# cirKITers/qml-essentials

Measured on AMD Instinct MI355X. Metric: gate_applies_per_s, higher is better.
Workload: dtype complex64

## Files before the change

### qml-essentials_amd/csrc/qmle_engine.hip

```cpp
#include <hip/hip_runtime.h>

#include <cmath>
#include <cstdio>
#include <cstdlib>
#include <cstring>
#include <algorithm>
#include <atomic>
#include <new>
#include <utility>

#include "qmle_internal.h"
#include "qmle_host.h"
#include "qmle_dev.h"
#include "qmle_matrices.h"

#include <map>
#include <mutex>
#include <vector>

namespace {

template <bool GMAJOR>
__global__ void __launch_bounds__(64)
k_build_matrices(const BuildOp *__restrict__ build, const BuildGroup *__restrict__ groups, int n_groups,
// ... 806 lines not shown
    const float *mats = d_mats + (size_t)b0 * plan->mat_floats;
    const float *ang = d_angles ? d_angles + (size_t)b0 * plan->n_slots : nullptr;
    float2 *cols = d_cols ? d_cols + (size_t)b0 * plan->fold_groups * 16 : nullptr;
    bool initialised = false;
    TileRoute route;
    for (size_t si = 0; si < plan->stages.size(); ++si) {
      const Stage &st = plan->stages[si];
      const ChunkPipeline::StageQueued stage_queued = pipe.begin_stage(chunk_no, si);
      ProfScope prof_scope(plan, (int)si, stream);
      if (st.kind == ST_TILE) {
        const bool last = si + 1 == plan->stages.size();
        const bool last_mw = fuse_mw && last, last_fused = !fuse_mw && fuse_expval && last;
        const TileBuffers tb{stc, mats, ang, last_mw || last_fused ? d_partial : nullptr, last_fused ? obs_masks : nullptr,
                             cols, d_coef + (size_t)b0 * 32};
        TileRequest rq;
        rq.batch = bc;
        rq.init_zero = !initialised;
        rq.meas = last_mw ? TM_STORE_MW : !last_fused ? TM_STORE : by_position ? TM_EXPVAL_PARTIAL : TM_EXPVAL_MASKS;
        rq.n_obs = last_fused ? n_obs : 0;
        rq.from_zero = true;
        rq.fold_cols = cols != nullptr;
        rq.multi_rows = last_mw || (last_fused && (oc.single_bits || rq.meas == TM_EXPVAL_MASKS));
        rq.semi_single = oc.semi_single;
        const bool reuse = !last_mw && si == 0 && reuse_zeros;
        if (reuse) rq.zeroed_states = slot_zeroed[slot];
        rc = launch_tile(plan, si, tb, rq, stream, &route);
        note_product_form(plan, si, route, meas_type);
        if (last_fused && !is_reg_measure(route.family)) {
          plan->last_run.measure_tpw = 1 << route.row_shift;
          plan->last_run.measure_regs = route.from_regs;
          plan->last_run.wave_private = route.wave_private;
          plan->last_run.staging_dma = (route.walk & kWalkDma) != 0;
          plan->last_run.lane_swap = (route.walk & kWalkLaneSwap) != 0;
        }
        if (reuse && route.fill) {
          slot_zeroed[slot] = bc;
          filled_states += (uint64_t)bc;
        }
        if (reuse && route.fill_elided) elided = true;
        initialised = true;
      } else {
        if (!initialised) {
          launch_init_zero(stc, n, bc, stream);
          initialised = true;
        }
        rc = run_stage_inplace(plan, st, stc, mats, ang, bc, stream);
      }
      if (rc != QMLE_OK) return rc;
    }
    if (!initialised) launch_init_zero(stc, n, bc, stream);
    if (meas_type == QMLE_MEAS_PROBS) {
      const uint64_t tc = (uint64_t)bc * (D / 2);
      launch_probs(stc, (float *)d_out + (size_t)b0 * D, tc, stream);
    } else if (meas_type == QMLE_MEAS_EXPVAL_Z && fuse_expval) {
      const bool reg_measure = is_reg_measure(route.family);
      const int tiles = (1 << (n - plan->stages.back().T)) >> route.row_shift;
      launch_expval_final((const float *)d_partial, tiles, bc, n_obs, by_position && !reg_measure ? oc.by_position : oc.by_index,
                          (float *)d_out + (size_t)b0 * n_obs, stream);
    } else if (meas_type == QMLE_MEAS_EXPVAL_Z) {
      rc = oc.single_bits
               ? run_expval(stc, n, bc, oc.by_position.bits, n_obs, (float *)d_out + (size_t)b0 * n_obs,
                            d_partial, L.partial_bytes, stream)
               : run_parity_pos(stc, n, bc, obs_masks, n_obs, (float *)d_out + (size_t)b0 * n_obs,
                                d_partial, L.partial_bytes, stream);
      if (rc != QMLE_OK) return rc;
    } else if (meas_type == QMLE_MEAS_MEYER_WALLACH) {
// ... 371 lines not shown
```

### qml-essentials_amd/csrc/qmle_host.h

```cpp
#pragma once
#include <hip/hip_runtime.h>

#include <cstddef>
#include <cstdint>

#include "qmle_internal.h"

namespace qmle {

struct ObsBits {
  int8_t bits[QMLE_MAX_QUBITS] = {};
  uint32_t row_mask[QMLE_MAX_QUBITS] = {};
};

enum TileMeas : int {
  TM_STORE = 0,
  TM_PROBS = 1,
  TM_EXPVAL = 2,
  TM_EXPVAL_PARTIAL = 3,
  TM_EXPVAL_MASKS = 4,
  TM_STORE_MW = 5,
  TM_MW_ONLY = 6,
};

// ... 52 lines not shown
int tile_threads(int T);
constexpr uint32_t kWalkSlab = 1u, kWalkSyncStaged = 2u, kWalkSyncTileEnd = 4u, kWalkDma = 8u, kWalkLaneSwap = 16u,
                   kWalkLaneSwapCross = 32u;
struct TileRequest {
  int batch = 1;
  bool init_zero = false;
  int meas = TM_STORE;
  int n_obs = 0;
  bool from_zero = false;
  bool fold_cols = false;
  bool multi_rows = false;
  int zeroed_states = 0;
  bool semi_single = false;
  bool no_multi_zin = false;
  bool no_mw_lean = false;
};
struct TileRoute {
  int status = QMLE_OK;
  TileFamily family = TF_TILE;
  bool dense4 = false, mw = false;
  bool measure = false, multi = false, ws = false, masks = false;
  int mono_q = 0;
  bool pair = false;
  bool nt = false;
  unsigned grid_x = 1, grid_y = 1, threads = 64;
  size_t lds_bytes = 0;
  bool compact = false;
  uint32_t tile_free = 0;
  bool mw_lean = false, slots_in_lds = false;
  bool fill = false, fill_elided = false;
  int tpw = 1, row_shift = 0;
  uint32_t walk = 0;
  bool from_regs = false, wave_private = false, product_form = false;
};
TileRoute route_tile(const qmle_plan *p, size_t stage, const TileRequest &rq);
struct TileBuffers {
  float2 *states = nullptr;
  const float *mats = nullptr, *angles = nullptr;
  void *out = nullptr;
  const uint32_t *obs_masks = nullptr;
  float2 *cols = nullptr;
  float *coef = nullptr;
};
int launch_tile(const qmle_plan *p, size_t stage, const TileBuffers &b, TileRequest rq, hipStream_t stream,
                TileRoute *taken = nullptr);

int launch_direct(const qmle_plan *p, const LoweredOp &op, float2 *states, const float *mats,
                  int batch, hipStream_t stream);
void launch_init_zero(float2 *states, int n, int batch, hipStream_t stream);
void launch_diag_all(float2 *states, int n, int batch, const float *marks, const float *angles,
                     int n_slots, int slot, hipStream_t stream);
void launch_fill_zero(float2 *states, uint64_t n_float4, hipStream_t stream);

int expval_blocks(int n);
int overlap_blocks(int n);
int run_expval(const float2 *states, int n, int batch, const int8_t *obs_bits, int n_obs,
               float *d_out, void *ws, size_t ws_bytes, hipStream_t stream);
int run_parity_pos(const float2 *states, int n, int batch, const uint32_t *pos_masks, int n_obs,
                   float *d_out, void *ws, size_t ws_bytes, hipStream_t stream);
void launch_expval_final(const float *partial, int n_rows, int batch, int n_obs, const ObsBits &ob,
                         float *d_out, hipStream_t stream);
void launch_probs(const float2 *states, float *d_out, uint64_t total_chunks, hipStream_t stream);
void launch_density(const float2 *states, float2 *d_out, int n, int batch, hipStream_t stream);
bool mw_fusable(int n, const Stage &last);
bool mw_lean(int n, const Stage &last);
bool mw_lean_layout(int n, const Stage &last);
// ... 26 lines not shown
```

### qml-essentials_amd/csrc/qmle_internal.h

```cpp
#pragma once
#include <cstdint>
#include <string>
#include <vector>

#include "qmle_sv.h"

namespace qmle {


enum LKind : uint8_t {
  LK_1Q = 0,
  LK_2Q = 1,
  LK_DIAG_ALL = 2,
  LK_4Q = 3
};
enum LFlag : uint8_t {
  LF_DIAG = 1,
  LF_PERMX = 2,
  LF_PHASE = 4,
};

enum GKind : uint8_t {
  GK_SWEEP = 0,
  GK_REG4 = 1,
// ... 117 lines not shown
};
static inline ZregRecord zreg_record(uint16_t r) {
  return {(uint32_t)r & 15u, ((uint32_t)r >> 4) & 63u, ((uint32_t)r >> 10) & 31u, (uint32_t)r >> 15};
}

struct StageProfile {
  bool on = false;
  std::vector<void *> start, stop;
  std::vector<int> stage;
  size_t used = 0;
};

struct DevicePlan {
  int device = -1;
  void *blob = nullptr;
  size_t blob_bytes = 0;
  LoweredOp *d_ops = nullptr;
  OpGroup *d_op_groups = nullptr;
  BuildOp *d_build = nullptr;
  BuildGroup *d_groups = nullptr;
  float *d_consts = nullptr;
  LoweredOp *d_ops2 = nullptr;
  Group2 *d_groups2 = nullptr;
  uint32_t *d_tbl2 = nullptr;
};

enum { kChunkLoopNone = 0, kChunkLoopOneStream, kChunkLoopStaged, kChunkLoopFree };
constexpr const char *kChunkLoopNames[] = {"none", "one_stream", "staged", "free"};

struct LastRun {
  uint64_t stage0_written = 0;
  int measure_tpw = 0;
  bool measure_regs = false, wave_private = false, staging_dma = false, lane_swap = false;
  int chunk_loop = kChunkLoopNone;
  uint64_t product_form_stages = 0;
  bool matrices_from_map = false;
  bool measured_form = false;
};

}

struct qmle_plan {
  int n = 0, n_slots = 0;
  unsigned flags = 0;
  std::vector<qmle_op> ops;
  std::vector<float> consts;
  std::vector<qmle::LoweredOp> lowered;
  std::vector<std::vector<int>> lowered_src;
  std::vector<qmle::LoweredOp> dev_ops;
  std::vector<int> dev_src;
  std::vector<qmle::OpGroup> op_groups;
  std::vector<qmle::LoweredOp> ops2;
  std::vector<uint8_t> ops2_perm_tail;
  std::vector<qmle::Group2> groups2;
  std::vector<uint32_t> tbl2;
  std::vector<qmle::BuildOp> build_ops;
  std::vector<qmle::BuildGroup> groups;
  int n_groups_needed = 0;
  int n_product_groups = 0;
  std::vector<qmle::Stage> stages;
  uint32_t mat_floats = 0;
  uint32_t mat_floats_unit = 0;
  uint32_t mat_floats_old = 0;
  int fold_groups = 0;
  double model_cost = 0.0;
  int chosen_candidate = -1;
// ... 58 lines not shown
```

### qml-essentials_amd/csrc/qmle_plan.cpp

```cpp
#include <algorithm>
#include <cstdio>
#include <cstdlib>
#include <cstring>
#include <cmath>
#include <functional>
#include <sstream>

#include "qmle_internal.h"

namespace qmle {

namespace {

struct OpInfo {
  int n_wires;
  int n_params;
  bool has_const;
};

bool op_info(int opcode, OpInfo *info) {
  switch (opcode) {
    case QMLE_OP_ID: case QMLE_OP_X: case QMLE_OP_Y: case QMLE_OP_Z:
    case QMLE_OP_H: case QMLE_OP_S:
      *info = {1, 0, false}; return true;
// ... 1783 lines not shown
    describe_measuring(os, p, s);
    if (st.kind == ST_TILE) {
      os << ",\"unit_form_ops\":[";
      for (size_t i = 0; i < st.unit_form_ops.size(); ++i) os << (i ? "," : "") << st.unit_form_ops[i];
      os << "],\"scale_carriers\":[";
      for (size_t i = 0; i < st.scale_carriers.size(); ++i) os << (i ? "," : "") << st.scale_carriers[i];
      os << "],\"fast_ops\":[";
      if (st.fast_ok && st.fast_end > st.fast_begin) {
        uint32_t k = p->groups2[st.fast_begin].op_begin;
        bool any = false;
        for (int g = st.fast_begin; g < st.fast_end; ++g)
          for (int j = 0; j < (int)p->groups2[g].n_ops; ++j, ++k, any = true)
            os << (any ? "," : "") << "[" << (int)p->ops2[k].pad << "," << p->ops2[k].mat_off << "]";
      }
      os << "],\"product_form_groups\":[";
      for (int g = st.fast_begin; g < st.fast_end; ++g)
        os << (g > st.fast_begin ? "," : "") << ((p->groups2[g].sync & kGroupProduct) ? "true" : "false");
      os << "],\"product_form_records\":[";
      for (int g = st.fast_begin; g < st.fast_end; ++g)
        os << (g > st.fast_begin ? "," : "") << ((p->groups2[g].sync & kGroupProduct) ? (long long)p->groups2[g].prod_off : -1ll);
      os << "],\"closing_free_groups\":[";
      for (int g = st.fast_begin; g < st.fast_end; ++g)
        os << (g > st.fast_begin ? "," : "") << ((p->groups2[g].sync & kGroupClosingFree) ? "true" : "false");
      os << "],\"group_product_form_last_run\":" << (s < 64 && ((p->last_run.product_form_stages >> s) & 1u) ? "true" : "false")
         << ",\"measured_form_last_run\":" << (s + 1 == p->stages.size() && p->last_run.measured_form ? "true" : "false");
    }
    if (s + 1 == p->stages.size())
      os << ",\"measure_tiles_per_workgroup_last_run\":" << p->last_run.measure_tpw
         << ",\"measured_from_registers_last_run\":" << (p->last_run.measure_regs ? "true" : "false")
         << ",\"wave_private_walk_last_run\":" << (p->last_run.wave_private ? "true" : "false")
         << ",\"staging_dma_last_run\":" << (p->last_run.staging_dma ? "true" : "false")
         << ",\"last_group_lane_swap_last_run\":" << (p->last_run.lane_swap ? "true" : "false")
         << ",\"chunk_loop_last_run\":\"" << kChunkLoopNames[p->last_run.chunk_loop] << "\""
         << ",\"matrices_from_map_last_run\":" << (p->last_run.matrices_from_map ? "true" : "false");
    os << ",\"src_ops\":[";
    for (size_t i = 0; i < st.src_ops.size(); ++i) os << (i ? "," : "") << st.src_ops[i];
    os << "]}";
  }
  os << "]";
  if (p->expval_child)
    os << ",\"absorbed_ops\":" << p->absorbed.size()
       << ",\"expval_plan\":" << describe_plan(p->expval_child);
  os << "}";
  return os.str();
}

}
```

### qml-essentials_amd/csrc/qmle_tile.hip

```cpp
#include <hip/hip_runtime.h>

#include <cmath>
#include <cstdio>
#include <cstdlib>
#include <cstring>
#include <algorithm>
#include <atomic>
#include <new>
#include <utility>

#include "qmle_internal.h"
#include "qmle_host.h"
#include "qmle_dev.h"
#include "qmle_tile_dev.h"

namespace {

template <bool DENSE4, bool MW = false>
__global__ void k_tile(const TileArgs a) {
  extern __shared__ float4 smem4[];
  float2 *s = reinterpret_cast<float2 *>(smem4);
  const int T = a.T, L = a.L;
  uint32_t *lut = reinterpret_cast<uint32_t *>(s + (1u << T));
  const uint32_t lut_n = (1u << (T - L)) < 4u ? 4u : (1u << (T - L));
// ... 854 lines not shown
  const int n_obs = a.n_obs;
  for (int k0 = 0; k0 < n_obs; k0 += 8) {
    float v[8];
#pragma unroll
    for (int k = 0; k < 8; ++k) {
      v[k] = 0.f;
      if (k0 + k < n_obs) {
        const uint32_t m = om[k0 + k];
        const uint32_t mu = (m >> (T - 3)) & 7u;
        float t = 0.f;
#pragma unroll
        for (int u = 0; u < 8; ++u) {
          const float d = (m & 1u) ? Df[u] : S[u];
          t += (__popc((uint32_t)u & mu) & 1) ? -d : d;
        }
        v[k] = (__popc((uint32_t)lane & (m >> 1) & 63u) & 1) ? -t : t;
      }
    }
    wave_sums_dpp63(v);
    if (lane == kWave - 1) {
#pragma unroll
      for (int k = 0; k < 8; ++k) red[(k0 + k) * nw + wv] = v[k];
    }
  }
  __syncthreads();
  if (tid < n_obs) {
    const uint32_t mw = om[tid] >> 7;
    float r = 0.f;
    for (int w = 0; w < nw; ++w) r += (__popc((uint32_t)w & mw) & 1) ? -red[tid * nw + w] : red[tid * nw + w];
    reinterpret_cast<float *>(a.out)[(size_t)b * n_obs + tid] = r;
  }
}

template <bool NT, bool MEASURE, bool MULTI, bool WS = false, bool MW = false, bool MASKS = false>
__global__ void __launch_bounds__(512) __attribute__((amdgpu_waves_per_eu(MASKS ? 4 : 5))) k_tile2(const TileArgs a, const Tile2Args f) {
  extern __shared__ float4 smem4[];
  float2 *s = reinterpret_cast<float2 *>(smem4);
  const int T = a.T;
  const uint32_t sbo = lds_offset_of(smem4);
  float *red = a.meas == TM_EXPVAL ? reinterpret_cast<float *>(s + (1u << T)) : reinterpret_cast<float *>(s);
  const int tid = threadIdx.x, nt = blockDim.x;
  const int b = blockIdx.y;
  const int tpw = MULTI ? f.tpw : 1;
  uint32_t tile = blockIdx.x * (uint32_t)tpw;
  if (!MULTI && a.compact) {
    uint32_t rest = tile, free_bits = a.tile_free;
    tile = 0;
    while (rest) {
      const uint32_t low = free_bits & (0u - free_bits);
      if (rest & 1u) tile |= low;
      free_bits ^= low;
      rest >>= 1;
    }
  }
  const uint32_t n_tiles = gridDim.x * (uint32_t)tpw;
  const size_t D = (size_t)1 << a.n;
  uint64_t base = tile2_base(a, f, tile);
  char *st = reinterpret_cast<char *>(a.states + (size_t)b * D + base);
  constexpr bool ZR = MEASURE && MULTI && !WS && !MW && !MASKS;
  const uint32_t walk = ZR ? f.walk : (kWalkSyncStaged | kWalkSyncTileEnd);
  const bool slab = ZR && (walk & kWalkSlab) != 0;
  const bool dma = ZR && (walk & kWalkDma) != 0;
  const uint32_t jl = slab ? (2u * (tid & (kWave - 1))) | ((uint32_t)(tid / kWave) << 10) : 2u * tid;
  const int ush = slab ? 7 : T - 3;
  uint32_t goff8;
  if (f.n_in_runs < 0) {
// ... 7 lines not shown
    goff8 = g << 3;
  }
  uint32_t uoff[8], soff[8];
#pragma unroll
  for (int u = 0; u < 8; ++u) {
    uoff[u] = f.uoff8[u];
    soff[u] = sw((uint32_t)u << ush) << 3;
  }
  const uint32_t sl = (sw(jl) << 3) + sbo;
  const float4 z4 = make_float4(0.f, 0.f, 0.f, 0.f);
  if (!MULTI && (a.init_zero ? base != 0 : (tile & a.zin_outer) != 0)) {
    if (MW) {
      if (a.meas == TM_STORE_MW) {
#pragma unroll
        for (int u = 0; u < 8; ++u) st4<NT>(reinterpret_cast<float4 *>(st + uoff[u] + goff8), z4);
      }
      float *po = reinterpret_cast<float *>(a.out) + ((size_t)b * n_tiles + tile) * kMwFusedRow;
      if (tid < kMwFusedRow) po[tid] = 0.f;
    } else if (!MEASURE && a.meas == TM_STORE) {
#pragma unroll
      for (int u = 0; u < 8; ++u) st4<NT>(reinterpret_cast<float4 *>(st + uoff[u] + goff8), z4);
    } else if (!MEASURE) {
      char *po = reinterpret_cast<char *>(reinterpret_cast<float *>(a.out) + (size_t)b * D + base);
#pragma unroll
      for (int u = 0; u < 8; ++u) *reinterpret_cast<float2 *>(po + (uoff[u] >> 1) + (goff8 >> 1)) = make_float2(0.f, 0.f);
    } else {
      float *po = reinterpret_cast<float *>(a.out) +
                  ((size_t)b * n_tiles + tile) * (QMLE_MAX_QUBITS + 1);
      if (tid <= QMLE_MAX_QUBITS) po[tid] = 0.f;
    }
    return;
  }
  auto dma_tile = [&](const char *p) {
    if constexpr (ZR) {
      const uint32_t wv = (uint32_t)__builtin_amdgcn_readfirstlane(tid / kWave);
      __attribute__((address_space(3))) char *slab0 =
          (__attribute__((address_space(3))) char *)reinterpret_cast<char *>(smem4) + (wv << 13);
      asm volatile("" : "+s"(p));
      uint32_t vo[4];
      static_for<4>([&](auto k) {
        vo[(int)k] = goff8 ^ f.dma_delta[(int)k];
        asm volatile("" : "+v"(vo[(int)k]));
      });
      static_for<8>([&](auto u) {
        const char *src = p + uoff[(int)u] + vo[(int)u & 3];
        __builtin_amdgcn_global_load_lds((const __attribute__((address_space(1))) void *)src, slab0 + ((int)u << 10), 16, 0,
                                         NT ? 2 : 0);
      });
    }
  };
  if (dma) dma_tile(st);
  const Group2 QMLE_CONSTANT *grp = as_constant(f.groups);
  const uint32_t addr = f.n_groups > 0 ? f.tbl[grp->tbl + tid] : 0u;
  const u64 QMLE_CONSTANT *mrow = as_constant(reinterpret_cast<const u64 *>(a.mats + (size_t)b * a.mat_floats));
  int qsrc = -1;
  if (MEASURE) {
    const int8_t QMLE_CONSTANT *ka = (const int8_t QMLE_CONSTANT *)__builtin_amdgcn_kernarg_segment_ptr();
    qsrc = tid <= QMLE_MAX_QUBITS ? (int)ka[offsetof(TileArgs, qsrc) + tid] : 64;
  }
  const bool plain = MULTI || (!a.init_zero && !a.zin_local);
  float4 v[8];
  const uint32_t zl_m = MULTI ? (a.zin_local & ~1u) : 0u;
  const bool z0_m = MULTI && (a.zin_local & 1u) != 0;
  auto load_tile = [&](const char *p) {
    if (MULTI && a.zin_local) {
#pragma unroll
      for (int u = 0; u < 8; ++u) {
        v[u] = z4;
        if (((jl | ((uint32_t)u << ush)) & zl_m) == 0) {
          v[u] = ld4<NT>(reinterpret_cast<const float4 *>(p + uoff[u] + goff8));
          if (z0_m) v[u].z = v[u].w = 0.f;
        }
      }
    } else {
#pragma unroll
      for (int u = 0; u < 8; ++u) v[u] = ld4<NT>(reinterpret_cast<const float4 *>(p + uoff[u] + goff8));
    }
  };
  if (plain && !ZR) load_tile(st);
  const uint32_t sl_outer = sl;
  float zsq[ZR ? 16 : 1], zwk[4] = {0.f, 0.f, 0.f, 0.f};
  if (ZR) static_for<16>([&](auto c) { zsq[ZR ? (int)c : 0] = 0.f; });
// ... 93 lines not shown
        }
      } else {
        float4 w[8];
#pragma unroll
        for (int u = 0; u < 8; ++u) w[u] = lds_ld128(sl ^ soff[u]);
#pragma unroll
        for (int u = 0; u < 8; ++u) st4<NT>(reinterpret_cast<float4 *>(st_cur + uoff[u] + goff8), w[u]);
      }
    } else {
      char *po = reinterpret_cast<char *>(reinterpret_cast<float *>(a.out) + (size_t)b * D + base_cur);
#pragma unroll
      for (int u = 0; u < 8; ++u) {
        const float4 w = lds_ld128(sl ^ soff[u]);
        *reinterpret_cast<float2 *>(po + (uoff[u] >> 1) + (goff8 >> 1)) =
            make_float2(w.x * w.x + w.y * w.y, w.z * w.z + w.w * w.w);
      }
    }
    if (ZR && !(walk & kWalkSyncTileEnd)) asm volatile("" ::: "memory");
    else if (i + 1 < tpw) __syncthreads();
  }
  if (MW)
    tile_mw_finish(macc, T, (uint32_t)tid, reinterpret_cast<float *>(s),
                   reinterpret_cast<float *>(a.out) + ((size_t)b * gridDim.x + blockIdx.x) * kMwFusedRow, a.mw_lean != 0);
  else if (MEASURE && MULTI && MASKS) {
    if constexpr (MASKS)
      tile_m_finish(reinterpret_cast<float *>(a.out), red, pacc, a.n_obs, m_ol, T, tid, nt, blockIdx.x, gridDim.x, b);
  } else if (MEASURE && MULTI) {
    if constexpr (ZR)
      tile_zr_finish(reinterpret_cast<float *>(a.out), red, zsq, zwk, m_ol, T, qsrc, tid, nt,
                     31 - __builtin_clz((unsigned)tpw), blockIdx.x, gridDim.x, b);
  }
}


template <bool FOLD>
__global__ void __launch_bounds__(1024) k_reg_measure(const TileArgs a, int q) {
  extern __shared__ float4 smem4[];
  OpSlot *slots = reinterpret_cast<OpSlot *>(smem4);
  uint32_t *meta = reinterpret_cast<uint32_t *>(slots + a.n_ops);
  uint32_t *m_thr = meta;
  uint32_t *m_reg = meta + 32;
  uint32_t *m_pack = meta + 64;
  uint32_t *flipF = meta + 68;
  uint32_t *flipP = meta + 100;
  float *red = reinterpret_cast<float *>(meta + 132);
  const int T = a.T, tid = threadIdx.x, b = blockIdx.y;
  const int n_outer = a.n - T;
  const OpGroup g = a.groups[0];
  const int b0 = g.bits[0], b1 = g.bits[1], b2 = g.bits[2], b3 = g.bits[3];

  tile_stage_slots(a, slots, b);
  if (tid < 32) {
    uint32_t mt = 0, mi = 0;
    if (tid < a.n_obs) {
      const uint32_t m = a.obs_mask[tid];
      int tb = 0;
      for (int j = 0; j < T; ++j) {
        const uint32_t bitv = (m >> a.tile_bits[j]) & 1u;
        if (j == b0) mi |= bitv;
        else if (j == b1) mi |= bitv << 1;
        else if (j == b2) mi |= bitv << 2;
        else if (j == b3) mi |= bitv << 3;
        else mt |= bitv << tb++;
      }
    }
    m_thr[tid] = mt;
// ... 496 lines not shown
}

namespace qmle {

size_t tile_lds_bytes(int T, int L, int n_slots) {
  const size_t lut_n = ((size_t)1 << (T - L)) < 4 ? 4 : ((size_t)1 << (T - L));
  return ((size_t)8 << T) + 4 * lut_n + 288 * sizeof(float) + (size_t)n_slots * sizeof(OpSlot);
}

int tile_threads(int T) {
  int t = T >= 4 ? 1 << (T - 4) : 64;
  if (t < 64) t = 64;
  if (t > 1024) t = 1024;
  return t;
}

#define QMLE_TILE2_INSTANCES(X)                    \
  X(false, false, false, false, false, false)      \
  X(true,  false, false, false, false, false)      \
  X(false, true,  false, false, false, false)      \
  X(true,  true,  false, false, false, false)      \
  X(false, false, true,  false, false, false)      \
  X(true,  false, true,  false, false, false)      \
  X(false, true,  true,  false, false, false)      \
  X(true,  true,  true,  false, false, false)      \
  X(false, true,  true,  false, false, true)       \
  X(true,  true,  true,  false, false, true)       \
  X(false, false, false, true,  false, false)      \
  X(false, true,  false, true,  false, false)      \
  X(false, true,  false, false, true,  false)      \
  X(true,  true,  false, false, true,  false)      \
  X(false, true,  false, true,  true,  false)
#define QMLE_TILE2(NT, ME, MU, WS, MW, MA) (k_tile2<NT, ME, MU, WS, MW, MA>)
#define QMLE_TILE_INSTANCES(X) X(false, false) X(true, false) X(false, true) X(true, true)
#define QMLE_TILE1(D4, MW) (k_tile<D4, MW>)

static TileRoute route_reg_measure(const qmle_plan *p, const Stage &st, TileFamily family, int batch) {
  TileRoute r;
  r.family = family;
  r.slots_in_lds = true;
  const int n_outer = p->n - st.T;
  int q = 0;
  while (q < 6 && q < n_outer && (((uint64_t)batch << n_outer) >> (q + 1)) >= 4096) ++q;
  r.threads = 1u << (st.T - 4);
  r.lds_bytes = (size_t)(st.op_end - st.op_begin) * sizeof(OpSlot) + (132 + 16 * 32 + 128) * sizeof(uint32_t);
  if (family == TF_REG_MEASURE_MONO) {
    q = 5;
    r.mono_q = 5;
    r.lds_bytes = 16 * 32 * sizeof(float);
    uint32_t zin_local = 0, zin_outer = 0;
    if (plan_sparse(p) && st.zero_in) stage_known_zeros(p, st, &zin_local, &zin_outer);
    const OpGroup &g = p->op_groups[st.grp_begin];
    if (g.bits[0] != 0 && st.tile_bits[0] == 0 && !(zin_local & 1u) && st.T >= 11 && n_outer >= 4) {
      q = 4;
      r.mono_q = 4;
      r.pair = true;
      r.threads = 1u << (st.T - 5);
      const int n_live = p->n - __builtin_popcount(st.zero_in);
      r.nt = ((uint64_t)batch << (n_live + 3)) >= (1ull << 30);
    }
  }
  r.grid_x = 1u << (n_outer - q);
  r.grid_y = (unsigned)batch;
  r.row_shift = q;
  r.tpw = 1 << q;
  return r;
}

TileRoute route_tile(const qmle_plan *p, size_t si, const TileRequest &rq) {
  const Stage &st = p->stages[si];
  const int meas = rq.meas, batch = rq.batch, n_obs = rq.n_obs;
  const bool init_zero = rq.init_zero;
  if ((meas == TM_EXPVAL_PARTIAL || meas == TM_EXPVAL_MASKS) && !init_zero && n_obs >= 1 && n_obs <= 32) {
    TileFamily k = expval_kernel_of(p, si, plan_sparse(p));
    if (k == TF_REG_MEASURE && rq.semi_single) k = TF_TILE;
    if (k != TF_TILE) return route_reg_measure(p, st, k, batch);
  }
  TileRoute r;
  const bool from_zero = rq.from_zero && plan_sparse(p);
  uint32_t zin_local = 0, zin_outer = 0;
  if (from_zero && st.zero_in && !init_zero) stage_known_zeros(p, st, &zin_local, &zin_outer);
  const int n_ops = st.op_end - st.op_begin;
  r.slots_in_lds = tile_lds_bytes(st.T, st.L, n_ops) <= 160 * 1024;
  r.nt = st.T < p->n && !(from_zero && st.zero_in) && !init_zero &&
         ((uint64_t)batch << (p->n + 3)) >= (1ull << 30);
  r.mw_lean = meas == TM_STORE_MW && !rq.no_mw_lean && mw_lean_layout(p->n, st);
  if ((meas == TM_STORE_MW || (meas == TM_STORE && !st.next_tile && !init_zero)) && st.T < p->n &&
      ((uint64_t)batch << (p->n + 3)) >= (1ull << 30))
    r.nt = true;
  for (int g = st.grp_begin; g < st.grp_end; ++g)
    r.dense4 |= p->op_groups[g].kind == GK_DENSE4 || p->op_groups[g].kind == GK_REG4X;
  const unsigned tiles = 1u << (p->n - st.T);
  const int threads = tile_threads(st.T);
  r.threads = (unsigned)threads;
  r.grid_x = tiles;
  r.grid_y = (unsigned)batch;
  if (init_zero && !from_zero && meas == TM_STORE && st.T < p->n && tiles > 1 &&
      (st.fast_ok || st.T == kLdsMaxQubits) && p->n <= 28 && threads == (1 << (st.T - 4))) {
    if (rq.zeroed_states >= batch) r.fill_elided = true;
// ... 58 lines not shown
        r.grid_x /= 2u;
      }
    }
    if ((meas == TM_EXPVAL_PARTIAL || meas == TM_EXPVAL_MASKS) && r.tpw > 1) {
      if (!rq.multi_rows || r.tpw > 8) {
        r.grid_x *= (unsigned)r.tpw;
        r.tpw = 1;
      } else {
        r.row_shift = 31 - __builtin_clz((unsigned)r.tpw);
      }
    }
    if (meas == TM_EXPVAL_PARTIAL && r.tpw > 1) {
      if (!st.zreg_ok) {
        r.status = QMLE_ERR_INTERNAL;
        return r;
      }
      r.from_regs = true;
      r.wave_private = st.wave_private;
      r.walk = (p->groups2[st.fast_begin].sync & 1 ? kWalkSyncStaged : 0u) | (st.sync_tile_end ? kWalkSyncTileEnd : 0u);
      if (st.slab_load) {
        r.walk |= kWalkSlab;
        const bool dma = walk_by_dma(st, zin_local);
        if (dma) r.walk |= kWalkDma;
        if (walk_by_lane_swap(st, dma)) r.walk |= kWalkLaneSwap | (st.lane_swap_cross ? kWalkLaneSwapCross : 0u);
      }
    }
    r.lds_bytes = ((size_t)8 << st.T) +
                  (meas == TM_EXPVAL ? (size_t)QMLE_MAX_QUBITS * (threads >= kWave ? threads / kWave : 1) * sizeof(float) : 0);
    r.measure = !(meas == TM_STORE || meas == TM_PROBS);
    r.multi = r.tpw > 1;
    r.mw = meas == TM_STORE_MW || meas == TM_MW_ONLY;
    r.ws = r.mw ? st.T == p->n : st.T == p->n && !r.multi && !r.nt;
    r.masks = !r.mw && !r.ws && r.measure && r.multi && meas == TM_EXPVAL_MASKS;
    return r;
  }
  r.lds_bytes = tile_lds_bytes(st.T, st.L, r.slots_in_lds ? n_ops : 0);
  if (meas == TM_STORE_MW || meas == TM_MW_ONLY) {
    if (st.T < 10 || threads != (1 << (st.T - 4))) {
      r.status = QMLE_ERR_UNSUPPORTED;
      return r;
    }
    r.mw = true;
  }
  return r;
}

namespace {

TileArgs route_tile_args(const qmle_plan *p, const Stage &st, const TileBuffers &b, const TileRequest &rq,
                         const TileRoute &r) {
  TileArgs a = fill_tile_args(p, st, b.states, b.mats, b.angles, rq.init_zero, rq.meas, b.out, b.obs_masks, rq.n_obs,
                              rq.from_zero && plan_sparse(p));
  a.slots_in_lds = r.slots_in_lds;
  a.nt = r.nt;
  a.mw_lean = r.mw_lean;
  a.compact = r.compact;
  a.tile_free = r.tile_free;
  return a;
}

int issue_reg_measure(const qmle_plan *p, const Stage &st, const TileBuffers &b, const TileRequest &rq,
                      const TileRoute &r, hipStream_t stream) {
  const int batch = rq.batch, n_obs = rq.n_obs, n_outer = p->n - st.T;
  TileArgs a = fill_tile_args(p, st, b.states, b.mats, b.angles, false, TM_EXPVAL_MASKS, b.out, b.obs_masks, n_obs,
                              plan_sparse(p));
  a.slots_in_lds = 1;
// ... 49 lines not shown
      for (int i = 0; i < 4; ++i)
        pa.gpos[g][i] = (uint32_t)st.tile_bits[p->op_groups[st.grp_begin + g].bits[i]];
    if (r.nt) hipLaunchKernelGGL(k_product_stream<true>, grid, block, 0, stream, pa);
    else hipLaunchKernelGGL(k_product_stream<false>, grid, block, 0, stream, pa);
  } else {
    const TileArgs a = route_tile_args(p, st, b, rq, r);
    const uint32_t n_tiles = r.compact ? 1u << __builtin_popcount(r.tile_free) : 1u << (p->n - st.T);
    hipLaunchKernelGGL(k_tile_product, grid, block, r.lds_bytes, stream, a, b.cols, r.tpw, n_tiles);
  }
  HIPCHK(hipGetLastError());
  return QMLE_OK;
}

int issue_tile(const qmle_plan *p, const Stage &st, const TileBuffers &b, const TileRequest &rq, const TileRoute &r,
               hipStream_t stream) {
  if (FirstUse once{0}; once.first) {
#define QMLE_X(D4, MW)                      \
  QMLE_LDS_BASE_CHECK(QMLE_TILE1(D4, MW)); \
  HIPCHK(hipFuncSetAttribute((const void *)QMLE_TILE1(D4, MW), hipFuncAttributeMaxDynamicSharedMemorySize, 160 * 1024));
    QMLE_TILE_INSTANCES(QMLE_X)
#undef QMLE_X
    once.done();
  }
  const TileArgs a = route_tile_args(p, st, b, rq, r);
  const dim3 grid(r.grid_x, r.grid_y), block(r.threads);
#define QMLE_X(D4, MW) \
  if (r.dense4 == D4 && r.mw == MW) hipLaunchKernelGGL(QMLE_TILE1(D4, MW), grid, block, r.lds_bytes, stream, a); else
  QMLE_TILE_INSTANCES(QMLE_X) return QMLE_ERR_INTERNAL;
#undef QMLE_X
  HIPCHK(hipGetLastError());
  return QMLE_OK;
}

int issue_tile2(const qmle_plan *p, const Stage &st, const TileBuffers &b, const TileRequest &rq, const TileRoute &r,
                hipStream_t stream) {
  if (FirstUse once{1}; once.first) {
#define QMLE_X(NT, ME, MU, WS, MW, MA)                      \
  QMLE_LDS_BASE_CHECK(QMLE_TILE2(NT, ME, MU, WS, MW, MA)); \
  HIPCHK(hipFuncSetAttribute((const void *)QMLE_TILE2(NT, ME, MU, WS, MW, MA), hipFuncAttributeMaxDynamicSharedMemorySize, 160 * 1024));
    QMLE_TILE2_INSTANCES(QMLE_X)
#undef QMLE_X
    once.done();
  }
  TileArgs a = route_tile_args(p, st, b, rq, r);
  Tile2Args f;
  f.groups = p->dev.d_groups2 + st.fast_begin;
  f.ops = p->dev.d_ops2;
  f.tbl = p->dev.d_tbl2;
  f.n_groups = st.fast_end - st.fast_begin;
  f.n_ops_stage = 0;
  for (int g = st.fast_begin; g < st.fast_end; ++g) f.n_ops_stage += p->groups2[g].n_ops;
  f.gtab = st.fast_gtab;
  {
    int nr = 0;
    const int n_outer = p->n - st.T;
    for (int i = 0; i < n_outer && nr <= 6;) {
      int len = 1;
      while (i + len < n_outer && st.outer_bits[i + len] == st.outer_bits[i] + len) ++len;
      if (nr < 6) {
        f.run_off[nr] = (uint32_t)i;
        f.run_mask[nr] = len >= 32 ? 0xffffffffu : ((1u << len) - 1u);
        f.run_pos[nr] = (uint32_t)st.outer_bits[i];
      }
      ++nr;
      i += len;
    }
    f.n_runs = nr <= 6 ? nr : -1;
    for (int k = nr < 6 ? nr : 6; k < 6; ++k) f.run_off[k] = f.run_mask[k] = f.run_pos[k] = 0;
  }
  auto lane_runs = [&](int top) { f.n_in_runs = stage_lane_runs(st, top, f.in_off, f.in_mask, f.in_pos); };
  lane_runs(st.T - 4);
  for (unsigned u = 0; u < 8; ++u)
    f.uoff8[u] = (((u & 1u) << st.tile_bits[st.T - 3]) | (((u >> 1) & 1u) << st.tile_bits[st.T - 2]) |
                  (((u >> 2) & 1u) << st.tile_bits[st.T - 1])) << 3;
  f.walk = r.walk;
  for (int k = 0; k < 4; ++k) f.dma_delta[k] = 0;
  f.tpw = r.tpw;
  f.tile_stride = r.tpw > 1 ? 1u << st.outer_bits[0] : 0u;
  if (r.from_regs) {
    static_assert(sizeof(st.zreg) <= sizeof(a.obs_local), "the records travel in TileArgs::obs_local");
    std::memcpy(a.obs_local, st.zreg, sizeof(st.zreg));
    for (int j = 0; j < st.T; ++j) a.qsrc[(int)st.tile_bits[j]] = (uint8_t)j;
    a.qsrc[QMLE_MAX_QUBITS] = (uint8_t)kZrTotal;
    if (r.walk & kWalkSlab) {
      f.gtab = st.fast_gtab_slab;
      lane_runs(st.T - 1);
      for (unsigned u = 0; u < 8; ++u)
        f.uoff8[u] = (((u & 1u) << st.tile_bits[7]) | (((u >> 1) & 1u) << st.tile_bits[8]) |
                      (((u >> 2) & 1u) << st.tile_bits[9])) << 3;
    }
    if (r.walk & kWalkDma) {
      f.gtab = st.fast_gtab_dma;
      for (int k = 0; k < 4; ++k) f.dma_delta[k] = st.dma_delta[k];
    }
    if (r.walk & kWalkLaneSwap) {
      static_assert(sizeof(st.zreg_swap) == sizeof(st.zreg), "one record layout");
      std::memcpy(a.obs_local, st.zreg_swap, sizeof(st.zreg_swap));
    }
  }
  const dim3 grid(r.grid_x, r.grid_y), block(r.threads);
#define QMLE_X(NT, ME, MU, WS, MW, MA)                                                                         \
  if (r.nt == NT && r.measure == ME && r.multi == MU && r.ws == WS && r.mw == MW && r.masks == MA)             \
    hipLaunchKernelGGL(QMLE_TILE2(NT, ME, MU, WS, MW, MA), grid, block, r.lds_bytes, stream, a, f);           \
  else
  QMLE_TILE2_INSTANCES(QMLE_X) return QMLE_ERR_INTERNAL;
#undef QMLE_X
  HIPCHK(hipGetLastError());
  return QMLE_OK;
}

}

int launch_tile(const qmle_plan *p, size_t stage, const TileBuffers &b, TileRequest rq, hipStream_t stream,
                TileRoute *taken) {
  const Stage &st = p->stages[stage];
  rq.no_multi_zin = std::getenv("QMLE_NO_MULTI_ZIN") != nullptr;
  rq.no_mw_lean = rq.meas == TM_STORE_MW && mw_no_lean_switch();
  const TileRoute r = route_tile(p, stage, rq);
  if (taken) *taken = r;
  if (r.status != QMLE_OK) return r.status;
  if (r.fill) launch_fill_zero(b.states, ((uint64_t)rq.batch << p->n) / 2u , stream);
  switch (r.family) {
    case TF_TILE: return issue_tile(p, st, b, rq, r, stream);
    case TF_TILE2: return issue_tile2(p, st, b, rq, r, stream);
    case TF_TILE_PRODUCT:
    case TF_PRODUCT_STREAM: return issue_product(p, st, b, rq, r, stream);
    default: return issue_reg_measure(p, st, b, rq, r, stream);
  }
}

}

int qmle_plan_tile_route(const qmle_plan *plan, int stage, int batch, int meas, int n_obs, unsigned request_flags,
                         char *buf, size_t cap) {
  using namespace qmle;
  if (!plan || stage < 0 || (size_t)stage >= plan->stages.size() || plan->stages[stage].kind != ST_TILE || batch < 1 ||
      batch > kMaxGridY || meas < TM_STORE || meas > TM_MW_ONLY || n_obs < 0 || n_obs > QMLE_MAX_QUBITS)
    return QMLE_ERR_INVALID_ARG;
  TileRequest rq;
  rq.batch = batch;
  rq.meas = meas;
  rq.n_obs = n_obs;
  rq.init_zero = request_flags & QMLE_ROUTE_INIT_ZERO;
  rq.from_zero = request_flags & QMLE_ROUTE_FROM_ZERO;
  rq.fold_cols = request_flags & QMLE_ROUTE_FOLD_COLS;
  rq.multi_rows = request_flags & QMLE_ROUTE_MULTI_ROWS;
  rq.zeroed_states = (request_flags & QMLE_ROUTE_ZEROS_IN_PLACE) ? batch : 0;
  rq.semi_single = request_flags & QMLE_ROUTE_SEMI_SINGLE;
  rq.no_multi_zin = request_flags & QMLE_ROUTE_NO_MULTI_ZIN;
  rq.no_mw_lean = request_flags & QMLE_ROUTE_NO_MW_LEAN;
  const TileRoute r = route_tile(plan, (size_t)stage, rq);
  auto tf = [](bool v) { return v ? "true" : "false"; };
  char js[1024];
  const int len = std::snprintf(
      js, sizeof(js),
      "{\"status\":%d,\"family\":\"%s\",\"dense4\":%s,\"mw\":%s,\"nt\":%s,\"measure\":%s,\"multi\":%s,\"ws\":%s,"
      "\"masks\":%s,\"mono_q\":%d,\"pair\":%s,\"grid\":[%u,%u],\"threads\":%u,\"lds_bytes\":%zu,\"compact\":%s,"
      "\"tile_free\":%u,\"mw_lean\":%s,\"slots_in_lds\":%s,\"fill\":%s,\"fill_elided\":%s,\"tiles_per_workgroup\":%d,"
      "\"row_shift\":%d,\"walk_slab\":%s,\"walk_sync_staged\":%s,\"walk_sync_tile_end\":%s,\"staging_dma\":%s,"
      "\"lane_swap\":%s,\"lane_swap_crossed\":%s,\"from_registers\":%s,\"wave_private\":%s,\"product_form\":%s}",
      r.status, kTileFamilyNames[r.family], tf(r.dense4), tf(r.mw), tf(r.nt), tf(r.measure), tf(r.multi), tf(r.ws),
      tf(r.masks), r.mono_q, tf(r.pair), r.grid_x, r.grid_y, r.threads, r.lds_bytes, tf(r.compact), r.tile_free,
      tf(r.mw_lean), tf(r.slots_in_lds), tf(r.fill), tf(r.fill_elided), r.tpw, r.row_shift, tf(r.walk & kWalkSlab),
      tf(r.walk & kWalkSyncStaged), tf(r.walk & kWalkSyncTileEnd), tf(r.walk & kWalkDma), tf(r.walk & kWalkLaneSwap),
      tf(r.walk & kWalkLaneSwapCross), tf(r.from_regs), tf(r.wave_private), tf(r.product_form));
  if (buf && cap > 0) {
    const size_t nc = (size_t)len < cap - 1 ? (size_t)len : cap - 1;
    std::memcpy(buf, js, nc);
    buf[nc] = 0;
  }
  return len;
}
```

Measured before the change: 4.005 million.

## Add specialized measure-walk kernel for DMA lane-swap register-measure tile stages

```diff
diff --git a/qml-essentials_amd/csrc/qmle_engine.hip b/qml-essentials_amd/csrc/qmle_engine.hip
--- a/qml-essentials_amd/csrc/qmle_engine.hip
+++ b/qml-essentials_amd/csrc/qmle_engine.hip
@@ -862,6 +862,7 @@
           plan->last_run.wave_private = route.wave_private;
           plan->last_run.staging_dma = (route.walk & kWalkDma) != 0;
           plan->last_run.lane_swap = (route.walk & kWalkLaneSwap) != 0;
+          plan->last_run.walk_kernel = route.walk_kernel;
         }
         if (reuse && route.fill) {
           slot_zeroed[slot] = bc;
diff --git a/qml-essentials_amd/csrc/qmle_host.h b/qml-essentials_amd/csrc/qmle_host.h
--- a/qml-essentials_amd/csrc/qmle_host.h
+++ b/qml-essentials_amd/csrc/qmle_host.h
@@ -108,6 +108,7 @@
   int tpw = 1, row_shift = 0;
   uint32_t walk = 0;
   bool from_regs = false, wave_private = false, product_form = false;
+  bool walk_kernel = false;
 };
 TileRoute route_tile(const qmle_plan *p, size_t stage, const TileRequest &rq);
 struct TileBuffers {
diff --git a/qml-essentials_amd/csrc/qmle_internal.h b/qml-essentials_amd/csrc/qmle_internal.h
--- a/qml-essentials_amd/csrc/qmle_internal.h
+++ b/qml-essentials_amd/csrc/qmle_internal.h
@@ -173,6 +173,7 @@
   uint64_t stage0_written = 0;
   int measure_tpw = 0;
   bool measure_regs = false, wave_private = false, staging_dma = false, lane_swap = false;
+  bool walk_kernel = false;
   int chunk_loop = kChunkLoopNone;
   uint64_t product_form_stages = 0;
   bool matrices_from_map = false;
diff --git a/qml-essentials_amd/csrc/qmle_plan.cpp b/qml-essentials_amd/csrc/qmle_plan.cpp
--- a/qml-essentials_amd/csrc/qmle_plan.cpp
+++ b/qml-essentials_amd/csrc/qmle_plan.cpp
@@ -1839,7 +1839,8 @@
          << ",\"staging_dma_last_run\":" << (p->last_run.staging_dma ? "true" : "false")
          << ",\"last_group_lane_swap_last_run\":" << (p->last_run.lane_swap ? "true" : "false")
          << ",\"chunk_loop_last_run\":\"" << kChunkLoopNames[p->last_run.chunk_loop] << "\""
-         << ",\"matrices_from_map_last_run\":" << (p->last_run.matrices_from_map ? "true" : "false");
+         << ",\"matrices_from_map_last_run\":" << (p->last_run.matrices_from_map ? "true" : "false")
+         << ",\"walk_kernel_last_run\":" << (p->last_run.walk_kernel ? "true" : "false");
     os << ",\"src_ops\":[";
     for (size_t i = 0; i < st.src_ops.size(); ++i) os << (i ? "," : "") << st.src_ops[i];
     os << "]}";
diff --git a/qml-essentials_amd/csrc/qmle_tile.hip b/qml-essentials_amd/csrc/qmle_tile.hip
--- a/qml-essentials_amd/csrc/qmle_tile.hip
+++ b/qml-essentials_amd/csrc/qmle_tile.hip
@@ -910,6 +910,25 @@
   }
 }
 
+template <bool NT>
+__device__ __forceinline__ void dma_tile_pieces(float4 *smem4, const char *p, int tid, uint32_t goff8,
+                                                const uint32_t (&uoff)[8], const uint32_t (&delta)[4]) {
+  const uint32_t wv = (uint32_t)__builtin_amdgcn_readfirstlane(tid / kWave);
+  __attribute__((address_space(3))) char *slab0 =
+      (__attribute__((address_space(3))) char *)reinterpret_cast<char *>(smem4) + (wv << 13);
+  asm volatile("" : "+s"(p));
+  uint32_t vo[4];
+  static_for<4>([&](auto k) {
+    vo[(int)k] = goff8 ^ delta[(int)k];
+    asm volatile("" : "+v"(vo[(int)k]));
+  });
+  static_for<8>([&](auto u) {
+    const char *src = p + uoff[(int)u] + vo[(int)u & 3];
+    __builtin_amdgcn_global_load_lds((const __attribute__((address_space(1))) void *)src, slab0 + ((int)u << 10), 16, 0,
+                                     NT ? 2 : 0);
+  });
+}
+
 template <bool NT, bool MEASURE, bool MULTI, bool WS = false, bool MW = false, bool MASKS = false>
 __global__ void __launch_bounds__(512) __attribute__((amdgpu_waves_per_eu(MASKS ? 4 : 5))) k_tile2(const TileArgs a, const Tile2Args f) {
   extern __shared__ float4 smem4[];
@@ -983,22 +1002,7 @@
     return;
   }
   auto dma_tile = [&](const char *p) {
-    if constexpr (ZR) {
-      const uint32_t wv = (uint32_t)__builtin_amdgcn_readfirstlane(tid / kWave);
-      __attribute__((address_space(3))) char *slab0 =
-          (__attribute__((address_space(3))) char *)reinterpret_cast<char *>(smem4) + (wv << 13);
-      asm volatile("" : "+s"(p));
-      uint32_t vo[4];
-      static_for<4>([&](auto k) {
-        vo[(int)k] = goff8 ^ f.dma_delta[(int)k];
-        asm volatile("" : "+v"(vo[(int)k]));
-      });
-      static_for<8>([&](auto u) {
-        const char *src = p + uoff[(int)u] + vo[(int)u & 3];
-        __builtin_amdgcn_global_load_lds((const __attribute__((address_space(1))) void *)src, slab0 + ((int)u << 10), 16, 0,
-                                         NT ? 2 : 0);
-      });
-    }
+    if constexpr (ZR) dma_tile_pieces<NT>(smem4, p, tid, goff8, uoff, f.dma_delta);
   };
   if (dma) dma_tile(st);
   const Group2 QMLE_CONSTANT *grp = as_constant(f.groups);
@@ -1158,6 +1162,114 @@
   }
 }
 
+struct WalkGroup {
+  uint32_t tbl;
+  uint32_t off[4];
+  uint32_t prod_off;
+  uint32_t flags;
+};
+struct WalkArgs {
+  const float2 *states;
+  const float *mats;
+  float *out;
+  const uint32_t *tbl;
+  uint32_t mat_floats;
+  int n, T, tpw;
+  uint32_t tile_stride;
+  int n_runs;
+  uint32_t run_off[6], run_mask[6], run_pos[6];
+  int n_in_runs;
+  uint32_t in_off[4], in_mask[4], in_pos[4], gtab;
+  uint32_t uoff8[8], dma_delta[4];
+  WalkGroup g[3];
+  uint32_t last_prod_off, last_low1;
+  uint16_t zreg[16];
+  uint8_t qsrc[QMLE_MAX_QUBITS + 1];
+};
+#define QMLE_WOFF(c, g) \
+  ((((c) & 1) ? (g).off[0] : 0u) ^ (((c) & 2) ? (g).off[1] : 0u) ^ (((c) & 4) ? (g).off[2] : 0u) ^ (((c) & 8) ? (g).off[3] : 0u))
+template <bool NT, int G, bool CROSS>
+__global__ void __launch_bounds__(512) __attribute__((amdgpu_waves_per_eu(5))) k_measure_walk(const WalkArgs w) {
+  static_assert(G >= 1 && G <= 3, "gathered groups");
+  extern __shared__ float4 smem4[];
+  const uint32_t sbo = lds_offset_of(smem4);
+  float *red = reinterpret_cast<float *>(smem4);
+  const int tid = threadIdx.x, nt = blockDim.x, b = blockIdx.y, T = w.T, tpw = w.tpw;
+  uint64_t base = 0;
+  {
+    const uint32_t tile = blockIdx.x * (uint32_t)tpw;
+#pragma unroll
+    for (int r = 0; r < 6; ++r)
+      if (r < w.n_runs) base |= (uint64_t)((tile >> w.run_off[r]) & w.run_mask[r]) << w.run_pos[r];
+  }
+  const char *st = reinterpret_cast<const char *>(w.states + ((size_t)b << w.n) + base);
+  uint32_t goff8;
+  if (w.n_in_runs < 0) {
+    goff8 = w.tbl[w.gtab + tid];
+  } else {
+    const uint32_t jg = sw((2u * (tid & (kWave - 1))) | ((uint32_t)(tid / kWave) << 10));
+    uint32_t g = 0;
+#pragma unroll
+    for (int r = 0; r < 4; ++r)
+      if (r < w.n_in_runs) g |= ((jg >> w.in_off[r]) & w.in_mask[r]) << w.in_pos[r];
+    goff8 = g << 3;
+  }
+  uint32_t uoff[8];
+#pragma unroll
+  for (int u = 0; u < 8; ++u) uoff[u] = w.uoff8[u];
+  dma_tile_pieces<NT>(smem4, st, tid, goff8, uoff, w.dma_delta);
+  uint32_t addr[G];
+  static_for<G>([&](auto k) { addr[(int)k] = (w.tbl[w.g[(int)k].tbl + tid] & ~7u) + sbo; });
+  const u64 QMLE_CONSTANT *mrow = as_constant(reinterpret_cast<const u64 *>(w.mats + (size_t)b * w.mat_floats));
+  const char QMLE_CONSTANT *ka = (const char QMLE_CONSTANT *)__builtin_amdgcn_kernarg_segment_ptr();
+  const int qsrc = tid <= QMLE_MAX_QUBITS ? (int)(uint8_t)ka[offsetof(WalkArgs, qsrc) + tid] : 64;
+  const uint16_t QMLE_CONSTANT *zr = (const uint16_t QMLE_CONSTANT *)(ka + offsetof(WalkArgs, zreg));
+  float zsq[16], zwk[4] = {0.f, 0.f, 0.f, 0.f};
+  static_for<16>([&](auto c) { zsq[(int)c] = 0.f; });
+  for (int i = 0; i < tpw; ++i) {
+    if (i > 0) st += w.tile_stride * sizeof(float2);
+    asm volatile("s_waitcnt vmcnt(0)" ::: "memory");
+    A16 r;
+    auto group = [&](auto k, const auto &g, bool sync_next) {
+      uint32_t ad = addr[(int)k];
+      asm volatile("" : "+v"(ad));
+#define QMLE_LD(c) r.v##c = lds_ld64(ad ^ QMLE_WOFF(c, g));
+      QMLE_X16(QMLE_LD)
+#undef QMLE_LD
+      if constexpr ((int)k + 1 == G) {
+        if (i + 1 < tpw) {
+          asm volatile("s_waitcnt lgkmcnt(0)" ::: "memory");
+          dma_tile_pieces<NT>(smem4, st + w.tile_stride * sizeof(float2), tid, goff8, uoff, w.dma_delta);
+        }
+      }
+      product_group(r, mrow + (g.prod_off >> 1), (g.flags & 1u) != 0);
+      if constexpr ((int)k + 1 < G) {
+        asm volatile("" : "+v"(ad));
+#define QMLE_ST(c) lds_st64(ad ^ QMLE_WOFF(c, g), r.v##c);
+        QMLE_X16(QMLE_ST)
+#undef QMLE_ST
+        if (sync_next) __syncthreads();
+        else asm volatile("" ::: "memory");
+      }
+    };
+    static_for<G>([&](auto k) {
+      if constexpr (G == 3) {
+        const WalkGroup QMLE_CONSTANT *kg = (const WalkGroup QMLE_CONSTANT *)(ka + offsetof(WalkArgs, g)) + (int)k;
+        asm volatile("" : "+s"(kg));
+        group(k, kg[0], (int)k + 1 < G && (kg[(int)k + 1 < G ? 1 : 0].flags & 2u) != 0);
+      } else {
+        group(k, w.g[(int)k], (int)k + 1 < G && (w.g[(int)k + 1 < G ? (int)k + 1 : 0].flags & 2u) != 0);
+      }
+    });
+    swap_lanes_45<CROSS>(r);
+    product_group(r, mrow + (w.last_prod_off >> 1), w.last_low1 != 0);
+    tile_zr_accumulate(r, i, zsq, zwk);
+    asm volatile("" ::: "memory");
+  }
+  tile_zr_finish(w.out, red, zsq, zwk, zr, T, qsrc, tid, nt, 31 - __builtin_clz((unsigned)tpw), blockIdx.x, gridDim.x, b);
+}
+#undef QMLE_WOFF
+
 
 template <bool FOLD>
 __global__ void __launch_bounds__(1024) k_reg_measure(const TileArgs a, int q) {
@@ -1720,6 +1832,10 @@
   X(true,  true,  false, false, true,  false)      \
   X(false, true,  false, true,  true,  false)
 #define QMLE_TILE2(NT, ME, MU, WS, MW, MA) (k_tile2<NT, ME, MU, WS, MW, MA>)
+#define QMLE_WALK_INSTANCES(X)                                                                       \
+  X(false, 1, false) X(true, 1, false) X(false, 2, false) X(true, 2, false) X(false, 3, false) X(true, 3, false) \
+  X(false, 1, true) X(true, 1, true) X(false, 2, true) X(true, 2, true) X(false, 3, true) X(true, 3, true)
+#define QMLE_WALK(NT, G, CR) (k_measure_walk<NT, G, CR>)
 #define QMLE_TILE_INSTANCES(X) X(false, false) X(true, false) X(false, true) X(true, true)
 #define QMLE_TILE1(D4, MW) (k_tile<D4, MW>)
 
@@ -1753,6 +1869,35 @@
   r.row_shift = q;
   r.tpw = 1 << q;
   return r;
+}
+
+static int stage_outer_runs(const qmle_plan *p, const Stage &st, uint32_t *off, uint32_t *mask, uint32_t *pos) {
+  int nr = 0;
+  const int n_outer = p->n - st.T;
+  for (int i = 0; i < n_outer && nr <= 6;) {
+    int len = 1;
+    while (i + len < n_outer && st.outer_bits[i + len] == st.outer_bits[i] + len) ++len;
+    if (nr < 6 && off && mask && pos) {
+      off[nr] = (uint32_t)i;
+      mask[nr] = len >= 32 ? 0xffffffffu : ((1u << len) - 1u);
+      pos[nr] = (uint32_t)st.outer_bits[i];
+    }
+    ++nr;
+    i += len;
+  }
+  if (off && mask && pos)
+    for (int k = nr < 6 ? nr : 6; k < 6; ++k) off[k] = mask[k] = pos[k] = 0;
+  return nr <= 6 ? nr : -1;
+}
+
+static bool walk_kernel_serves(const qmle_plan *p, const Stage &st, const TileRoute &r, uint32_t zin_local) {
+  if (r.family != TF_TILE2 || !r.from_regs || !(r.walk & kWalkDma) || !(r.walk & kWalkLaneSwap)) return false;
+  if ((r.walk & (kWalkSyncStaged | kWalkSyncTileEnd)) || zin_local != 0 || r.tpw < 2) return false;
+  const int gathered = st.fast_end - st.fast_begin - 1;
+  if (gathered < 1 || gathered > 3) return false;
+  for (int g = st.fast_begin; g < st.fast_end; ++g)
+    if (!(p->groups2[g].sync & kGroupProduct) || (g + 2 < st.fast_end && p->groups2[g].relayout)) return false;
+  return stage_outer_runs(p, st, nullptr, nullptr, nullptr) >= 0;
 }
 
 TileRoute route_tile(const qmle_plan *p, size_t si, const TileRequest &rq) {
@@ -1877,6 +2022,7 @@
     r.mw = meas == TM_STORE_MW || meas == TM_MW_ONLY;
     r.ws = r.mw ? st.T == p->n : st.T == p->n && !r.multi && !r.nt;
     r.masks = !r.mw && !r.ws && r.measure && r.multi && meas == TM_EXPVAL_MASKS;
+    r.walk_kernel = walk_kernel_serves(p, st, r, zin_local);
     return r;
   }
   r.lds_bytes = tile_lds_bytes(st.T, st.L, r.slots_in_lds ? n_ops : 0);
@@ -1992,6 +2138,61 @@
   return QMLE_OK;
 }
 
+int issue_walk(const qmle_plan *p, const Stage &st, const TileArgs &a, const Tile2Args &f, const TileRoute &r,
+               hipStream_t stream) {
+  if (FirstUse once{2}; once.first) {
+#define QMLE_X(NT, G, CR)                      \
+  QMLE_LDS_BASE_CHECK(QMLE_WALK(NT, G, CR)); \
+  HIPCHK(hipFuncSetAttribute((const void *)QMLE_WALK(NT, G, CR), hipFuncAttributeMaxDynamicSharedMemorySize, 160 * 1024));
+    QMLE_WALK_INSTANCES(QMLE_X)
+#undef QMLE_X
+    once.done();
+  }
+  WalkArgs w;
+  std::memset(&w, 0, sizeof(w));
+  w.states = a.states;
+  w.mats = a.mats;
+  w.out = reinterpret_cast<float *>(a.out);
+  w.tbl = f.tbl;
+  w.mat_floats = a.mat_floats;
+  w.n = a.n;
+  w.T = a.T;
+  w.tpw = f.tpw;
+  w.tile_stride = f.tile_stride;
+  w.n_runs = stage_outer_runs(p, st, w.run_off, w.run_mask, w.run_pos);
+  w.n_in_runs = f.n_in_runs;
+  w.gtab = f.gtab;
+  std::memcpy(w.in_off, f.in_off, sizeof(w.in_off));
+  std::memcpy(w.in_mask, f.in_mask, sizeof(w.in_mask));
+  std::memcpy(w.in_pos, f.in_pos, sizeof(w.in_pos));
+  std::memcpy(w.uoff8, f.uoff8, sizeof(w.uoff8));
+  std::memcpy(w.dma_delta, f.dma_delta, sizeof(w.dma_delta));
+  const int gathered = st.fast_end - st.fast_begin - 1;
+  for (int k = 0; k < gathered && k < 3; ++k) {
+    const Group2 &g = p->groups2[st.fast_begin + k];
+    w.g[k].tbl = g.tbl;
+    for (int j = 0; j < 4; ++j) w.g[k].off[j] = g.off[1 << j];
+    w.g[k].prod_off = g.prod_off;
+    w.g[k].flags = ((g.sync & kGroupProductLow1) ? 1u : 0u) | ((g.sync & 1) ? 2u : 0u);
+  }
+  const Group2 &last = p->groups2[st.fast_end - 1];
+  w.last_prod_off = last.prod_off;
+  w.last_low1 = (last.sync & kGroupProductLow1) ? 1u : 0u;
+  static_assert(sizeof(w.zreg) <= sizeof(a.obs_local) && sizeof(w.qsrc) == sizeof(a.qsrc), "the records of TileArgs");
+  std::memcpy(w.zreg, a.obs_local, sizeof(w.zreg));
+  std::memcpy(w.qsrc, a.qsrc, sizeof(w.qsrc));
+  const bool cross = (r.walk & kWalkLaneSwapCross) != 0;
+  const dim3 grid(r.grid_x, r.grid_y), block(r.threads);
+#define QMLE_X(NT, G, CR)                                                          \
+  if (r.nt == NT && gathered == G && cross == CR && w.n_runs >= 0)                 \
+    hipLaunchKernelGGL(QMLE_WALK(NT, G, CR), grid, block, r.lds_bytes, stream, w); \
+  else
+  QMLE_WALK_INSTANCES(QMLE_X) return QMLE_ERR_INTERNAL;
+#undef QMLE_X
+  HIPCHK(hipGetLastError());
+  return QMLE_OK;
+}
+
 int issue_tile2(const qmle_plan *p, const Stage &st, const TileBuffers &b, const TileRequest &rq, const TileRoute &r,
                 hipStream_t stream) {
   if (FirstUse once{1}; once.first) {
@@ -2011,23 +2212,7 @@
   f.n_ops_stage = 0;
   for (int g = st.fast_begin; g < st.fast_end; ++g) f.n_ops_stage += p->groups2[g].n_ops;
   f.gtab = st.fast_gtab;
-  {
-    int nr = 0;
-    const int n_outer = p->n - st.T;
-    for (int i = 0; i < n_outer && nr <= 6;) {
-      int len = 1;
-      while (i + len < n_outer && st.outer_bits[i + len] == st.outer_bits[i] + len) ++len;
-      if (nr < 6) {
-        f.run_off[nr] = (uint32_t)i;
-        f.run_mask[nr] = len >= 32 ? 0xffffffffu : ((1u << len) - 1u);
-        f.run_pos[nr] = (uint32_t)st.outer_bits[i];
-      }
-      ++nr;
-      i += len;
-    }
-    f.n_runs = nr <= 6 ? nr : -1;
-    for (int k = nr < 6 ? nr : 6; k < 6; ++k) f.run_off[k] = f.run_mask[k] = f.run_pos[k] = 0;
-  }
+  f.n_runs = stage_outer_runs(p, st, f.run_off, f.run_mask, f.run_pos);
   auto lane_runs = [&](int top) { f.n_in_runs = stage_lane_runs(st, top, f.in_off, f.in_mask, f.in_pos); };
   lane_runs(st.T - 4);
   for (unsigned u = 0; u < 8; ++u)
@@ -2058,6 +2243,7 @@
       std::memcpy(a.obs_local, st.zreg_swap, sizeof(st.zreg_swap));
     }
   }
+  if (r.walk_kernel) return issue_walk(p, st, a, f, r, stream);
   const dim3 grid(r.grid_x, r.grid_y), block(r.threads);
 #define QMLE_X(NT, ME, MU, WS, MW, MA)                                                                         \
   if (r.nt == NT && r.measure == ME && r.multi == MU && r.ws == WS && r.mw == MW && r.masks == MA)             \
@@ -2118,12 +2304,14 @@
       "\"masks\":%s,\"mono_q\":%d,\"pair\":%s,\"grid\":[%u,%u],\"threads\":%u,\"lds_bytes\":%zu,\"compact\":%s,"
       "\"tile_free\":%u,\"mw_lean\":%s,\"slots_in_lds\":%s,\"fill\":%s,\"fill_elided\":%s,\"tiles_per_workgroup\":%d,"
       "\"row_shift\":%d,\"walk_slab\":%s,\"walk_sync_staged\":%s,\"walk_sync_tile_end\":%s,\"staging_dma\":%s,"
-      "\"lane_swap\":%s,\"lane_swap_crossed\":%s,\"from_registers\":%s,\"wave_private\":%s,\"product_form\":%s}",
+      "\"lane_swap\":%s,\"lane_swap_crossed\":%s,\"from_registers\":%s,\"wave_private\":%s,\"product_form\":%s,"
+      "\"walk_kernel\":%s}",
       r.status, kTileFamilyNames[r.family], tf(r.dense4), tf(r.mw), tf(r.nt), tf(r.measure), tf(r.multi), tf(r.ws),
       tf(r.masks), r.mono_q, tf(r.pair), r.grid_x, r.grid_y, r.threads, r.lds_bytes, tf(r.compact), r.tile_free,
       tf(r.mw_lean), tf(r.slots_in_lds), tf(r.fill), tf(r.fill_elided), r.tpw, r.row_shift, tf(r.walk & kWalkSlab),
       tf(r.walk & kWalkSyncStaged), tf(r.walk & kWalkSyncTileEnd), tf(r.walk & kWalkDma), tf(r.walk & kWalkLaneSwap),
-      tf(r.walk & kWalkLaneSwapCross), tf(r.from_regs), tf(r.wave_private), tf(r.product_form));
+      tf(r.walk & kWalkLaneSwapCross), tf(r.from_regs), tf(r.wave_private), tf(r.product_form),
+      tf(r.walk_kernel));
   if (buf && cap > 0) {
     const size_t nc = (size_t)len < cap - 1 ? (size_t)len : cap - 1;
     std::memcpy(buf, js, nc);
```

Result: faster. 4.142 million, median of 6 (+3.4%).
